# claserken/SISS

Hardware: AMD Instinct MI355X
Metric: unlearning samples/sec (= unlearning-steps/sec x batch x gpus), CelebA-HQ-256 DDPM SISS (higher is better)
Workload: dtype bf16; 1 GPU; delete_celeb.yaml: CelebA-HQ 256x256 DDPM UNet (113.7M params), SISS lambd=0.5, t=999, bf16, bs=16/GPU, GA=1, scaling_norm=500, AdamW lr 5e-6; loss_fn=importance_sampling_with_mixture, global_batch=16, grad_accum=1, parallelism=dp1, hipgraph=True

## Files before the change

### include/siss_hip.h

```cpp
#ifndef SISS_HIP_H
#define SISS_HIP_H
#include <stdint.h>
#ifdef __cplusplus
extern "C" {
#endif

typedef struct siss_tn_job {
    const void* Y; long ldy; const void* X; long ldx; float* dW; long set_stride;
    int N, C, npanels, nsets, rows_per_set, row_begin, row_end, nsplits;
    long x_set_rows;
    const void* zero_page; float* dbias; float* dbias2;
    int shifts[9]; int coffs[9];
    long bias_set_stride;
} siss_tn_job;

typedef struct siss_rk_terms {
    const double* row[8]; double c[8]; int n;
} siss_rk_terms;

long siss_loss_partials_words(int B, long chw);
int siss_mixture_fwd(const void* x0, const void* a0, const void* noise, int in_bf16, const int64_t* t, const
    float* u, const float* alphas_cumprod, const float* gamma_tab, const float* sigma_tab, float lambd, int B,
    long chw, void* x_mix, float* gamma_t, float* sigma_t, float* dist_x, float* dist_a, float* iw_x, float* iw_a,
    double* partials, void* stream);
// ... 71 lines not shown
int siss_groupnorm_set_slab(int on);
long siss_gn_partial_words(int n, int H, int W, int C, int G);
int siss_quad_stats(const void* x, long ld, int M, int N, int rows_per_image, float* qs, void* stream);
int siss_groupnorm_fwd_qs(const void* x, const float* gamma, const float* beta, void* y, float* mean, float*
    rstd, float* partial, const float* qsA, int ca, const float* qsB, int N, int H, int W, int C, int G, float
    eps, int silu, int out_compact, int ldx, void* stream);
int siss_groupnorm_fwd_ld(const void* x, const float* gamma, const float* beta, void* y, float* mean, float*
    rstd, float* partial, int N, int H, int W, int C, int G, float eps, int silu, int out_compact, int ldx, void*
    stream);
int siss_groupnorm_fwd(const void* x, const float* gamma, const float* beta, void* y, float* mean, float*
    rstd, float* partial, int N, int H, int W, int C, int G, float eps, int silu, int out_compact, void* stream);
int siss_groupnorm_bwd_ld(const void* dy, const void* x, const float* gamma, const float* beta, const float*
    mean, const float* rstd, void* dx, const void* accum, const void* accum2, void* dx2, int split_c, int
    accumulate2, float* dgamma, float* dbeta, float* colsum, long colsum_ld, float* partial, int n2, int nx, int
    set_images, long set_stride, int H, int W, int C, int G, int silu, int dy_compact, int ldx, void* stream);
int siss_groupnorm_bwd_ld_s2d(const void* dy, const void* x, const float* gamma, const float* beta, const
    float* mean, const float* rstd, void* dx, const void* accum, const void* accum2, void* dx2, int split_c, int
    accumulate2, float* dgamma, float* dbeta, float* colsum, long colsum_ld, float* partial, int n2, int nx, int
    set_images, long set_stride, int H, int W, int C, int G, int silu, int dy_compact, int ldx, void* stream);
int siss_groupnorm_bwd(const void* dy, const void* x, const float* gamma, const float* beta, const float*
    mean, const float* rstd, void* dx, const void* accum, const void* accum2, void* dx2, int split_c, int
    accumulate2, float* dgamma, float* dbeta, float* colsum, long colsum_ld, float* partial, int n2, int nx, int
    set_images, long set_stride, int H, int W, int C, int G, int silu, int dy_compact, void* stream);

int siss_conv_out_fprop(const void* x, const float* w, const float* bias, float* pred, int B, int H, int W,
    int C, int CO, void* stream);
int siss_conv_out_dgrad(const float* c, const float* w, void* dx, int N2, int H, int W, int C, int CO, void*
    stream);
int siss_conv_out_wgrad(const float* c, const void* x, float* dW, float* dbias, int nsets, int set_images, int
    nx, long set_stride_w, long set_stride_b, int H, int W, int C, int CO, void* stream);
int siss_conv_in_dgrad(const void* dh, long ld, const void* w, int kp, float* dx, int N, int Cin, int H, int
    W, int C0, void* stream);
int siss_conv_in_dgrad_f32(const void* dh, long ld, const void* w, int kp, float* dx, int N, int Cin, int H,
    int W, int C0, void* stream);

int siss_softmax_fwd(const void* s, void* p, long rows, int S, void* stream);
int siss_softmax_bwd(const void* p, const void* dp, void* ds, long rows, long p_rows, int S, float scale,
    void* stream);
int siss_mha_small_takes(int S, int D, int training);
int siss_mha_small_fwd(const void* q, const void* k, const void* v, void* o, float* lse, int N, int S, int C,
    int D, float scale, void* stream);
int siss_mha_small_bwd(const void* q, const void* k, const void* v, const void* o, const float* lse, const
    void* dout, void* dq, void* dk, void* dv, int n2, int nx, int S, int C, int D, float scale, void* stream);
int siss_mha_small_fwd_f32(const void* q, const void* k, const void* v, void* o, float* lse, int N, int S, int
    C, int D, float scale, void* stream);
int siss_mha_small_bwd_f32(const void* q, const void* k, const void* v, const void* o, const float* lse, const
// ... 225 lines not shown
```

### siss_amd/csrc/common.h

```cpp
#pragma once
#include <hip/hip_runtime.h>
#include <stdint.h>

typedef uint16_t bf16_t;

typedef __attribute__((ext_vector_type(8))) short bf16x8_t;
typedef __attribute__((ext_vector_type(4))) float f32x4_t;
typedef __attribute__((ext_vector_type(16))) float f32x16_t;
typedef __attribute__((ext_vector_type(4))) uint32_t u32x4_t;
typedef __attribute__((ext_vector_type(2))) uint32_t u32x2_t;
typedef __attribute__((ext_vector_type(2))) float f32x2_t;
typedef __attribute__((ext_vector_type(2))) __bf16 bf16x2_t;

#define SISS_OK 0
#define SISS_ERR_ARG 1
#define SISS_ERR_LAUNCH 2

#define SISS_CHECK_ARG(cond) \
    do {                     \
        if (!(cond)) return SISS_ERR_ARG; \
    } while (0)

#define SISS_LAUNCH_RET()                                 \
    do {                                                  \
// ... 85 lines not shown
__device__ __forceinline__ unsigned lds_addr(const void* p) {
    return (unsigned)(size_t)(__attribute__((address_space(3))) const char*)p;
}

static inline int cdiv(long a, long b) { return (int)((a + b - 1) / b); }

constexpr int kMaxDevices = 64;
constexpr int kQsTileRows = 254, kQsHalfRows = 128;
static inline int siss_current_device() {
    int dev = 0;
    return hipGetDevice(&dev) == hipSuccess && dev >= 0 && dev < kMaxDevices ? dev : -1;
}
static inline int siss_ensure_smem(const void* kernel, int bytes, unsigned char (&done)[kMaxDevices]) {
    const int dev = siss_current_device();
    if (dev < 0) return SISS_ERR_LAUNCH;
    if (!__atomic_load_n(&done[dev], __ATOMIC_ACQUIRE)) {
        if (hipFuncSetAttribute(kernel, hipFuncAttributeMaxDynamicSharedMemorySize, bytes) != hipSuccess) return SISS_ERR_LAUNCH;
        __atomic_store_n(&done[dev], (unsigned char)1, __ATOMIC_RELEASE);
    }
    return SISS_OK;
}

enum SissKernelId { SISS_K_NT = 0, SISS_K_NT_C3P, SISS_K_FLASH_FWD, SISS_K_FLASH_BWD, SISS_K_NT_SPLITK, SISS_K_TN1, SISS_K_TN3,
                    SISS_K_GN_SLAB, SISS_K_GN_QSTATS, SISS_K_FLASH_QSPLIT, SISS_K_ATTN1H_FWD, SISS_K_ATTN1H_BWD, SISS_K_TN_PAIR, SISS_K_FLASH32, SISS_K_FLASH32_FWD, SISS_K_NT_WIDE, SISS_K_COUNT };
void siss_count_dispatch(int kernel_id);
void* siss_workspace(long* bytes);
```

### siss_amd/csrc/groupnorm.hip

```cpp
#include "common.h"

namespace {

constexpr int kStatsDepth = 2;
constexpr int kThreads = 256;
constexpr int kMaxG = 32;
constexpr int kMaxC = 1024;

struct GNShape {
    int H, W, C, G, cpg, lpp, ppi;
    int chunk_px, nchunks;
    int ld, Gf, nslices;
    int ldx;
};

__device__ __forceinline__ long compact_row(int n, int pi, int H, int W) { return (long)n * H * W + pi; }

__device__ __forceinline__ void unpack8(u32x4_t r, float (&v)[8]) {
#pragma unroll
    for (int j = 0; j < 4; ++j) {
        v[2 * j] = __builtin_bit_cast(float, r[j] << 16);
        v[2 * j + 1] = __builtin_bit_cast(float, r[j] & 0xffff0000u);
    }
}
// ... 338 lines not shown
            }
        }
    }
    for (int k = 0; k < SETS; ++k) {
        reduce_slots(a1[k], active, slot, cc, s, red, ch1);
        reduce_slots(a2[k], active, slot, cc, s, red, ch2);
        const int n2 = k * nx + n;
        if (tid < 2 * s.G) {
            const int g = tid >> 1;
            const float* src = (tid & 1) ? ch2 : ch1;
            float t = 0.f;
            for (int c = g * s.cpg; c < (g + 1) * s.cpg; ++c) t += src[c] * gamma[c];
            partial[(((long)n2 * s.nslices + blockIdx.z) * s.nchunks + chunk) * 2 * s.G + tid] = t;
        }
        const long so = (long)(n2 / set_images) * set_stride + c0;
        for (int i = tid; i < s.C; i += kThreads) {
            atomicAdd(dgamma + so + i, ch2[i]);
            atomicAdd(dbeta + so + i, ch1[i]);
        }
        __syncthreads();
    }
}

template <bool SILU, int SETS, bool S2D>
__global__ __launch_bounds__(kThreads) void gn_bwd_apply_kernel(
    const bf16_t* __restrict__ dy, const bf16_t* __restrict__ x, const float* __restrict__ gamma,
    const float* __restrict__ beta, const float* __restrict__ mean, const float* __restrict__ rstd,
    const float* __restrict__ partial, GNShape s, int nx, int dy_compact, const bf16_t* __restrict__ accum,
    const bf16_t* __restrict__ accum2, bf16_t* __restrict__ dx, bf16_t* __restrict__ dx2, int split_c,
    int accumulate2, float* __restrict__ colsum, long colsum_ld, int pchunks) {
    __shared__ float sh_s1[SETS][kMaxG], sh_s2[SETS][kMaxG];
    __shared__ __attribute__((aligned(16))) float red[2048];
    __shared__ float chs[kMaxC];
    const int n = blockIdx.y, chunk = blockIdx.x, tid = threadIdx.x;
    const int c0 = blockIdx.z * s.C, g0 = blockIdx.z * s.G;
    gamma += c0; beta += c0;
    {
        __shared__ float fr[4][64];
        const double cnt = (double)s.H * s.W * s.cpg;
        for (int k = 0; k < SETS; ++k) {
            const int n2 = k * nx + n;
            fold_slab(partial + ((long)n2 * s.nslices + blockIdx.z) * pchunks * 2 * s.G, pchunks, s.G, fr);
            if (tid < s.G) {
                sh_s1[k][tid] = (float)(((double)fr[0][2 * tid] + fr[1][2 * tid] + fr[2][2 * tid] + fr[3][2 * tid]) / cnt);
                sh_s2[k][tid] = (float)(((double)fr[0][2 * tid + 1] + fr[1][2 * tid + 1] + fr[2][2 * tid + 1] + fr[3][2 * tid + 1]) / cnt);
            }
// ... 49 lines not shown
            const unsigned ooff = __umul24(q.row(), ob);
#pragma unroll
            for (int k = 0; k < SETS; ++k) {
                o.d[k] = ld16(dbase[k], doff);
                if (accum) o.a[k] = ld16(abase[k], roff);
                if (accum2) o.b[k] = ld16(bbase[k], roff);
                if (any_oacc) o.c[k] = oacc ? ld16(obase[k], ooff) : u32x4_t{0u, 0u, 0u, 0u};
            }
        };
        PixelWalk w(s, chunk, slot);
        int yy = S2D ? w.pi / s.W : 0;
        const int dyi = S2D ? s.ppi / s.W : 0;
        In nxt;
        if (w.ok()) issue(w, nxt);
        while (w.ok()) {
            const In cur = nxt;
            const unsigned ooff = out_off(w.row(), yy, w.x);
            if (S2D) yy += dyi + (w.x + w.dx >= s.W ? 1 : 0);
            w.next();
            if (w.ok()) issue(w, nxt);
            float v[8], xh[8], dsl[8];
            unpack8(cur.x, v);
#pragma unroll
            for (int e = 0; e < 8; ++e) {
                xh[e] = v[e] * rs[e] - mr[e];
                dsl[e] = (SILU ? dsilu_f(xh[e] * ga[e] + be[e]) : 1.f) * ga[e];
            }
#pragma unroll
            for (int k = 0; k < SETS; ++k) {
                float d[8], o[8];
                unpack8(cur.d[k], d);
#pragma unroll
                for (int e = 0; e < 8; ++e) {
                    const float t = rs[e] * (d[e] * dsl[e] - m1[k][e] - xh[e] * m2[k][e]);
                    cs[k][e] += t;
                    o[e] = t;
                }
                if (accum) {
                    float r[8];
                    unpack8(cur.a[k], r);
#pragma unroll
                    for (int e = 0; e < 8; ++e) o[e] += r[e];
                }
                if (accum2) {
                    float r[8];
                    unpack8(cur.b[k], r);
#pragma unroll
                    for (int e = 0; e < 8; ++e) o[e] += r[e];
                }
                if (any_oacc) {
                    float r[8];
                    unpack8(cur.c[k], r);
#pragma unroll
                    for (int e = 0; e < 8; ++e) o[e] += r[e];
                }
                st16(obase[k], ooff, pack8(o));
            }
        }
    }
    if (colsum) {
        for (int k = 0; k < SETS; ++k) {
            reduce_slots(cs[k], active, slot, cc, s, red, chs);
            for (int i = tid; i < s.C; i += kThreads) atomicAdd(colsum + (long)(k * nx + n) * colsum_ld + c0 + i, chs[i]);
            __syncthreads();
        }
    }
}

constexpr int kBlocksFwd = 768, kBlocksBwd = 512, kBlocksBwdStats = 767;

bool make_shape(int H, int W, int C, int G, GNShape& s, int N = 16, int blocks = kBlocksFwd) {
    if (H <= 0 || W <= 0 || C <= 0 || G <= 0 || G > kMaxG || C % G || C % 8) return false;
    s.H = H; s.W = W; s.ld = C; s.ldx = C; s.Gf = G; s.cpg = C / G;
    int gs = G;
    if (C > kMaxC) {
        int best = 0, best_util = -1;
        gs = 0;
        for (int d = G; d >= 1; --d) {
            if (G % d) continue;
            const int cs = d * s.cpg;
            if (cs > kMaxC || cs % 8) continue;
            const int lpp = cs / 8, util = (kThreads / lpp) * lpp;
            if (util * 10 >= kThreads * 9) { gs = d; break; }
            if (util > best_util) { best_util = util; best = d; }
        }
        if (gs == 0) gs = best;
        if (gs == 0) return false;
// ... 140 lines not shown
                          float* dbeta, float* colsum, long colsum_ld, float* partial, int n2, int nx, int set_images,
                          long set_stride, int H, int W, int C, int G, int silu, int dy_compact, int ldx, void* stream) {
    return gn_bwd_launch(dy, x, gamma, beta, mean, rstd, dx, accum, accum2, dx2, split_c, accumulate2, dgamma, dbeta, colsum, colsum_ld,
                         partial, n2, nx, set_images, set_stride, H, W, C, G, silu, dy_compact, ldx, 0, stream);
}
int siss_groupnorm_bwd_ld_s2d(const void* dy, const void* x, const float* gamma, const float* beta,
                              const float* mean, const float* rstd, void* dx, const void* accum, const void* accum2,
                              void* dx2, int split_c, int accumulate2, float* dgamma,
                              float* dbeta, float* colsum, long colsum_ld, float* partial, int n2, int nx, int set_images,
                              long set_stride, int H, int W, int C, int G, int silu, int dy_compact, int ldx, void* stream) {
    return gn_bwd_launch(dy, x, gamma, beta, mean, rstd, dx, accum, accum2, dx2, split_c, accumulate2, dgamma, dbeta, colsum, colsum_ld,
                         partial, n2, nx, set_images, set_stride, H, W, C, G, silu, dy_compact, ldx, 1, stream);
}
int siss_groupnorm_bwd(const void* dy, const void* x, const float* gamma, const float* beta,
                       const float* mean, const float* rstd, void* dx, const void* accum, const void* accum2,
                       void* dx2, int split_c, int accumulate2, float* dgamma,
                       float* dbeta, float* colsum, long colsum_ld, float* partial, int n2, int nx, int set_images,
                       long set_stride, int H, int W, int C, int G, int silu, int dy_compact, void* stream) {
    return siss_groupnorm_bwd_ld(dy, x, gamma, beta, mean, rstd, dx, accum, accum2, dx2, split_c, accumulate2, dgamma, dbeta,
                                 colsum, colsum_ld, partial, n2, nx, set_images, set_stride, H, W, C, G, silu, dy_compact, 0,
                                 stream);
}

}
```

### siss_amd/lib.py

```python
import ctypes as C
import os
import re
import threading

import torch

from . import prof

_HERE = os.path.dirname(os.path.abspath(__file__))
LIB_PATH = os.environ.get("SISS_LIB_PATH") or os.path.join(_HERE, "libsiss_hip.so")

P, I, L, D = C.c_void_p, C.c_int, C.c_long, C.c_double
HEADER = os.path.join(os.path.dirname(_HERE), "include", "siss_hip.h")
_SCALARS = {"int": C.c_int, "long": C.c_long, "float": C.c_float, "double": C.c_double}


def parse_prototypes(text):
    text = " ".join(re.sub(r"/\*.*?\*/", " ", text, flags=re.S).split())
    out = {}
    for ret, name, params in re.findall(r"\b(int|long) (siss_\w+) ?\(([^()]*)\) ?;", text):
        out[name] = (_SCALARS[ret], [])
        for decl in ([] if params.strip() in ("", "void") else params.split(",")):
            m = re.fullmatch(r"(?:const )?(\w+)( ?\* ?| )(\w+)", decl.strip())
            if m and "*" in m.group(2):
# ... 32 lines not shown
_MODE = threading.local()


def in_f32_mode():
    return bool(getattr(_MODE, "f32", False))


class f32_mode:

    def __init__(self, on):
        self.on = bool(on)

    def __enter__(self):
        self.prev, _MODE.f32 = getattr(_MODE, "f32", False), self.on
        return self

    def __exit__(self, *exc):
        _MODE.f32 = self.prev
        return False


KERNEL_IDS = {"gemm_nt_kernel": 0, "gemm_nt_c3p_kernel": 1, "flash_attn_fwd": 2, "flash_attn_bwd": 3,
              "gemm_nt_kernel/splitk": 4, "gemm_tn_kernel<1>": 5, "gemm_tn_kernel<3>": 6, "gn_slab": 7, "gn_qstats": 8, "flash_dkdv_qsplit": 9,
              "attn1h_fwd": 10, "attn1h_bwd": 11, "gemm_tn_pair": 12, "flash32_bwd": 13, "flash32_fwd": 14, "gemm_nt_kernel/wide": 15}


def dispatch_counts(reset=False):
    lib = load()
    out = {k: int(lib.siss_dispatch_count(i)) for k, i in KERNEL_IDS.items()}
    if reset:
        lib.siss_dispatch_reset()
    return out



class TNJob(C.Structure):
    _fields_ = [("Y", P), ("ldy", L), ("X", P), ("ldx", L), ("dW", P), ("set_stride", L),
                ("N", I), ("C", I), ("npanels", I), ("nsets", I), ("rows_per_set", I), ("row_begin", I), ("row_end", I),
                ("nsplits", I), ("x_set_rows", L), ("zero_page", P), ("dbias", P), ("dbias2", P),
                ("shifts", I * 9), ("coffs", I * 9), ("bias_set_stride", L)]


class RkTerms(C.Structure):
    _fields_ = [("row", P * 8), ("c", D * 8), ("n", I)]

    @classmethod
    def of(cls, pairs):
# ... 129 lines not shown
```

### siss_amd/prof.py

```python


def _true_rows(M, rows_per_image, Hp, Wp):
    if Hp > 2 and Wp > 2 and M % rows_per_image == 0:
        return (M // rows_per_image) * (Hp - 2) * (Wp - 2)
    return M


def _triples(shifts, coffs, n):
    return n % 3 == 0 and all(shifts[3 * g + 1] == shifts[3 * g] + 1 and shifts[3 * g + 2] == shifts[3 * g] + 2
                              and coffs[3 * g] == coffs[3 * g + 1] == coffs[3 * g + 2] for g in range(n // 3))


def _nt(a, N=None, npanels=1, batch=1, conv=False, planes=False):
    M, N, Kp = a["M"], a["N"] if N is None else N, a["Kp"]
    rpi, Hp, Wp = (a["rows_per_image"], a["Hp"], a["Wp"]) if conv else (1, 0, 0)
    c3p = (conv and not planes and npanels == 9 and batch == 1 and Kp % 64 == 0 and N % 128 == 0 and rpi >= 256
           and -(-M // 128) * -(-N // 128) >= 256 and _triples(a["shifts"], a["coffs"], 9))
    key = ("M", M, "N", N, "K", Kp, "panels", npanels, "batch", batch) + (("4 planes",) if planes else ())
    return ("siss_gemm_nt", 2.0 * _true_rows(M, rpi, Hp, Wp) * N * Kp * npanels * batch, key,
            "gemm_nt_c3p_kernel" if c3p else "gemm_nt_kernel", None)


def _nt_shortcut(a, outer, inner, folded, tag):
    rows = _true_rows(a["M"], a["rows_per_image"], a["Hp"], a["Wp"])
# ... 26 lines not shown

def _tn_pair(a):
    j3, j1 = _job(a["job3"]._obj), _job(a["job1"]._obj)
    key = ("N", j3["N"], "C", j3["C"], "panels", j3["npanels"], "+ N", j1["N"], "C", j1["C"], "panels", j1["npanels"],
           "rows", j3["row_end"] - j3["row_begin"])
    return None, _tn_flops(j3) + _tn_flops(j1), key, "gemm_tn_mixed_kernel", None


def _attn(products, heads, Sq, Sk, D, one_head=False):
    key = ("B", heads, "S", Sq, "D", D) if one_head else ("BH", heads, "Sq", Sq, "Sk", Sk, "D", D)
    return None, 2.0 * products * heads * Sq * Sk * D, key, None, None


def _gn_fwd(a, name="siss_groupnorm_fwd_ld"):
    return name, 0.0, ("n", a["N"], "H", a["H"], "C", a["C"]), name, 2.0 * 2 * a["N"] * a["H"] * a["W"] * a["C"]


def _gn_bwd(a, name="siss_groupnorm_bwd_ld"):
    passes = 2 + (a["accum"] is not None) + (a["accum2"] is not None)
    return (name, 0.0, ("n2", a["n2"], "H", a["H"], "C", a["C"]), name,
            2.0 * (a["H"] * a["W"] * a["C"]) * (a["nx"] + passes * a["n2"]))


def _hbm(nbytes):
    return None, 0.0, (), None, nbytes


def _conv_nt(a):
    return _nt(a, npanels=a["npanels"], conv=True)


_RULES = {
    "siss_gemm_nt": lambda a: _nt(a, npanels=a["npanels"], batch=a["batch"], conv=True),
    "siss_gemm_nt_qstats": _conv_nt,
    "siss_gemm_nt_d2s": _conv_nt,
    "siss_gemm_nt_d2s_bias": _conv_nt,
    "siss_gemm_nt_d2s_phases": lambda a: _nt(a, npanels=a["phase_p0"][4], conv=True, planes=True),
    "siss_gemm_nt_alpha_cols": _nt,
    "siss_gemm_nt_geglu_bwd": _nt,
    "siss_gemm_nt_geglu_fwd": lambda a: _nt(a, N=2 * a["F"]),
    "siss_conv3x3_sc": lambda a: _nt_shortcut(a, "N", "Kp", "K2", "+1x1 K"),
    "siss_conv3x3_dgrad_sc": lambda a: _nt_shortcut(a, "Kp", "N", "Nx", "+1x1 N"),
    "siss_gemm_nt_mulsub": lambda a: (None, 2.0 * a["M"] * a["N"] * a["Kp"] * a["batch"], (), "gemm_nt_kernel", None),
    "siss_gemm_tn": _tn,
    "siss_gemm_tn_bs": _tn,
    "siss_gemm_tn_grouped": lambda a: _tn_table(a, "gemm_tn_grouped_kernel"),
    "siss_gemm_tn_grouped_capped": lambda a: _tn_table(a, "gemm_tn_grouped_capped_kernel"),
    "siss_gemm_tn_pair": _tn_pair,
    "siss_attn1h_fwd": lambda a: _attn(2, a["B"], a["S"], a["S"], a["D"], one_head=True),
    "siss_attn1h_bwd": lambda a: _attn(5, a["nb"], a["S"], a["S"], a["D"], one_head=True),
    "siss_flash_attn_fwd": lambda a: _attn(2, a["BH"], a["Sq_pad"], a["valid_k"], a["D_pad"]),
    "siss_flash_attn_bwd": lambda a: _attn(5, a["nBH"], a["Sq_pad"], a["valid_k"], a["D_pad"]),
    "siss_flash_attn_fwd_merged": lambda a: _attn(2, a["B"] * a["H"], a["Sq"], a["Sk"], a["D"]),
    "siss_flash_attn_bwd_merged": lambda a: _attn(5, a["nB"] * a["H"], a["Sq"], a["Sk"], a["D"]),
    "siss_groupnorm_fwd": lambda a: _gn_fwd(a, None),
    "siss_groupnorm_fwd_ld": _gn_fwd,
    "siss_groupnorm_fwd_qs": _gn_fwd,
    "siss_groupnorm_bwd": lambda a: _gn_bwd(a, None),
    "siss_groupnorm_bwd_ld": _gn_bwd,
    "siss_groupnorm_bwd_ld_s2d": _gn_bwd,
    "siss_recombine_clip_adamw": lambda a: _hbm(32.0 * a["n"]),
    "siss_mixture_fwd": lambda a: _hbm(4.0 * (2 if a["in_bf16"] else 4) * a["B"] * a["chw"]),
    "siss_loss_bwd_seed": lambda a: _hbm((4 + 3 * (2 if a["in_bf16"] else 4) + 8.0) * a["B"] * a["chw"]),
}


def account(name, a):
    booked, work, key, symbol, nbytes = _RULES[name](a) if name in _RULES else (None, 0.0, (), None, None)
    base = booked or name
    base = base[:-3] if base.endswith("_ld") else base
    return base[:-7] if base.endswith("_merged") else base, work, key, symbol or booked or name, nbytes
```

### siss_amd/unet.py

```python
import math
from dataclasses import dataclass
from types import SimpleNamespace

import torch

from . import lib, ops
from .config import UNet2DConfig
from .layout import Act, ActView

ALIGN = 64


@dataclass
class PSpec:
    name: str
    kind: str
    ref_shape: tuple
    native_shape: tuple
    off: int
    numel: int


class ParamStore:

# ... 84 lines not shown
            if n not in sd:
                continue
            t = sd[n]
            if tuple(t.shape) != sp.ref_shape:
                raise ValueError(f"{n}: shape {tuple(t.shape)} != {sp.ref_shape}")
            self.flat[sp.off:sp.off + sp.numel] = self.to_native(sp, t.to(self.flat.device)).reshape(-1)

    def state_dict(self):
        return {n: self.from_native(sp, self.flat[sp.off:sp.off + sp.numel]).cpu() for n, sp in self.specs.items()}

    def grads_ref(self, which):
        return {n: self.from_native(sp, self.grads[which, sp.off:sp.off + sp.numel]).cpu()
                for n, sp in self.specs.items()}

    def flat_to_ref(self, flat):
        return {n: self.from_native(sp, flat[sp.off:sp.off + sp.numel]).cpu() for n, sp in self.specs.items()}


class UNetEngine:
    epi_stats = True
    d2s_epilogue = True
    direct_cat = True
    fold_shortcut = True
    subpixel_up = True
    subpixel_min_px = 1024
    subpixel_queue = 1
    side_max_batch = 1 << 30
    quad_stats = True
    phase_launch = True
    s2d_from_gn = True
    group_rows = 280000
    group_max = 42
    group_attn = True
    fused_attn = True
    wgrad_side = True
    side_blocks = 128
    side_max_px = 256
    side_follow = 1
    prep_side = True
    pair_top = True
    wgrad_overwrite = False
    fill_grads = True
    sparse_fill = True
    sparse_min_floats = 16384
    pair_min_rows = 280000

    def __init__(self, cfg: UNet2DConfig, device="cuda", dtype=torch.bfloat16, f32_fused=False):
        lib.load()
        self.cfg = cfg
        self.device = torch.device(device)
        assert dtype in (torch.bfloat16, torch.float32)
        self.adt, self.f32 = dtype, dtype == torch.float32
        self.f32_fused = bool(f32_fused) and self.f32
        if self.f32:
            self.epi_stats = False
            if not self.f32_fused:
                self.d2s_epilogue = self.fold_shortcut = False
                self.group_rows = 0
        if self.device.type == "cuda":
            lib.ensure_workspace(self.device)
        self.ps = ParamStore()
        self._declare_params()
        self.ps.relayout(self._grads_final_early)
        self.ps.allocate(self.device, f32=self.f32)
        self._build_temb_tables()
        self.wT = {}
        self._wds = {}
        self._acts = {}
        self._bufs = {}
        self._pool = {}
        self.tape = []
        self.gmap = {}
        self._uid = 0
        self.on_early_grads_final = None
        self._wq, self._held, self._held_release = [], {}, []
        self._pair1 = []
        self._wq_post = []
        self._side, self._side_busy, self._side_held, self._side_release, self._side_mark = None, False, {}, [], None
# ... 374 lines not shown
            yptr = y.data
        ldx = getattr(x, "ld", x.c)
        qa = qb = None
        ca = x.c
        if self.epi_stats:
            parts = getattr(x, "cat_parts", None)
            form = (x.c // G) % 4 == 0 and x.c % G == 0
            if parts is not None:
                sa = self._quad_stats_of(parts[0], form and parts[1].c <= 512 and parts[1].c % 8 == 0)
                sb = self._quad_stats_of(parts[1], form and sa is not None)
                if sa is not None and sb is not None:
                    qa, qb, ca = sa, sb, parts[0].c
            else:
                qa = self._quad_stats_of(x, form)
        if qa is not None:
            lib.call("siss_groupnorm_fwd_qs", x.data, ps.p(pre + ".weight"), ps.p(pre + ".bias"), yptr, mean, rstd,
                     self._gn_partial(x.n, x.h, x.w, x.c), qa, ca, qb, x.n, x.h, x.w, x.c, G, float(eps), int(silu),
                     int(compact_out), 0 if ldx == x.c else ldx)
        else:
            lib.call("siss_groupnorm_fwd_ld", x.data, ps.p(pre + ".weight"), ps.p(pre + ".bias"), yptr, mean, rstd,
                     self._gn_partial(x.n, x.h, x.w, x.c), x.n, x.h, x.w, x.c, G, float(eps), int(silu), int(compact_out),
                     0 if ldx == x.c else ldx)

        def bwd(dy, colsum=None, accum: Act = None, colsum_ld=0, accum2: Act = None, split=None):
            nb = self.nb
            held = accum is not None and self._is_held(accum.buf)
            if accum is not None and not held:
                self._wsync(accum)
            s2d = False
            if split is not None:
                da, db, accb = split[:3]
                s2d = len(split) > 3 and bool(split[3])
                dx, dx2p, split_c = da, db.data, (da.c // 4 if s2d else da.c)
                self._wsync(db)
            else:
                dx = accum if (accum is not None and not held) else self._get(nb, x.h, x.w, x.c)
                dx2p, split_c, accb = None, 0, False
            dyp = dy.data if isinstance(dy, Act) else dy
            lib.call("siss_groupnorm_bwd_ld_s2d" if s2d else "siss_groupnorm_bwd_ld", dyp, x.data, ps.p(pre + ".weight"), ps.p(pre + ".bias"), mean, rstd,
                     dx.data, accum.data if accum is not None else None,
                     accum2.data if accum2 is not None else None, dx2p, split_c, int(accb),
                     ps.g(pre + ".weight", self.gbase), ps.g(pre + ".bias", self.gbase), colsum, colsum_ld,
                     self._gn_partial(nb, x.h, x.w, x.c), nb, x.n, self.set_images, ps.total,
                     x.h, x.w, x.c, G, int(silu), int(not isinstance(dy, Act)), 0 if ldx == x.c else ldx)
            if held and split is None:
                self._put(accum)
            return dx
        return y, bwd

    def conv(self, x: Act, pre, ksize=3, rowbias=None, residual: Act = None, out_name=None, ldrb=None, cat_with=None,
             skip_head=None, want_stats=False, shortcut=None, fprop=True):
        ps = self.ps
        w = ps.sh(pre + ".weight")
        if ksize == 1:
            w = w.view(1, *w.shape)
        co = w.shape[1]
        if not fprop:
            y = None
        elif cat_with is not None and self.direct_cat:
            assert (cat_with.n, cat_with.h, cat_with.w) == (x.n, x.h, x.w)
            if isinstance(cat_with, ActView):
# ... 142 lines not shown

    def resnet(self, x: Act, pre, cat_with=None, skip_head=None):
        ps = self.ps
        cin = x.c
        cout = ps.specs[pre + ".conv1.weight"].ref_shape[0]
        B = x.n
        a1, gn1_b = self.gn(x, pre + ".norm1", True)
        col0, _ = self.temb_cols[pre]
        h, c1_b = self.conv(a1, pre + ".conv1", rowbias=self.tp_all[:, col0:], ldrb=self.temb_ntot, want_stats=True)
        a2, gn2_b = self.gn(h, pre + ".norm2", True)
        has_sc = cin != cout
        if has_sc:
            _, sc_b = self.conv(x, pre + ".conv_shortcut", ksize=1, fprop=False)
            out, c2_b = self.conv(a2, pre + ".conv2", cat_with=cat_with, skip_head=skip_head, want_stats=True,
                                  shortcut=(x, pre + ".conv_shortcut"))
        else:
            out, c2_b = self.conv(a2, pre + ".conv2", residual=x, cat_with=cat_with, skip_head=skip_head, want_stats=True)

        def bwd():
            nb = self.nb
            dout = self._take(out)
            gb = self.gbase
            acc_sc = None
            if has_sc:
                sc_b(dout, bias_grad=False, need_dx=False)
                da2, acc_sc = c2_b(dout, bias_grad2=ps.g(pre + ".conv_shortcut.bias", gb),
                                   sc_dgrad=(pre + ".conv_shortcut", x.c, lambda: self._get(nb, x.h, x.w, x.c)))
            else:
                da2 = c2_b(dout)
            dh = gn2_b(da2, colsum=self.dtp_all[:, col0:], accum=None, colsum_ld=self.temb_ntot)
            self._put(da2)
            da1 = c1_b(dh, bias_grad=False)
            self._put(dh)
            prior = self.gmap.pop(id(x), None)
            if has_sc:
                acc = acc_sc if acc_sc is not None else sc_b(dout, bias_grad=False, wgrad=False)
                self._put(dout)
            else:
                acc = dout
            parts = getattr(x, "cat_parts", None)
            if parts is not None:
                a, b = parts
                s2d = bool(getattr(a, "s2d_cot", False)) and self.gmap.get(id(a)) is None
                da = self._get(nb, a.h // 2, a.w // 2, 4 * a.c) if s2d else self._get(nb, a.h, a.w, a.c)
                accb = self.gmap.get(id(b))
                db = accb if accb is not None else self._get(nb, b.h, b.w, b.c)
                gn1_b(da1, accum=acc, accum2=prior, split=(da, db, accb is not None, s2d))
                self.gmap[id(b)] = db
                self._put(acc)
                self._give(a, da)
                x.cat_done = True
            else:
                dx = gn1_b(da1, accum=acc, accum2=prior)
                self.gmap[id(x)] = dx
            self._put(prior)
            self._put(da1)
        self.tape.append(bwd)
        return out

    def attention(self, x: Act, pre):
        ps = self.ps
        C, B, S = x.c, x.n, x.h * x.w
        D = self.cfg.head_dim(C)
        if (self.fused_attn and not self.f32 and D == C and x.w % 4 == 0 and not isinstance(x, ActView)
                and lib.query("siss_attn1h_takes", S, C)):
            return self._attention_fused(x, pre)
        small = D != C
        assert not small or D in (8, 16, 32), f"attention_head_dim {D} is not covered by the HIP kernels"
        if small:
            self._mha_check(S, D, training=False)
            self._mha_sites.append((S, D))
        scale = D ** -0.5
        rows = B * S
        nm = self._name(pre)
        hn, gn_b = self.gn(x, pre + ".group_norm", False, compact_out=True)
        bb = lambda s, shape: self._buf(nm + s, shape, self.adt)
        q, k, v = bb(".q", (rows, C)), bb(".k", (rows, C)), bb(".v", (rows, C))
# ... 514 lines not shown
        plan = None
        if sparse_key is not None and self.sparse_fill and self.wgrad_overwrite and not self.f32 and lib.has("siss_zero_ranges"):
            sparse_key = (sparse_key,) + self._wgrad_sig()
            self._fill_key = sparse_key
            plan = self._fill_plan = self._fill_plans.get(sparse_key)
        g = self.ps.grads

        def fill():
            if plan is None:
                g.zero_()
            elif plan["n"]:
                lib.call("siss_zero_ranges", g, plan["table"], plan["n"], plan["granules"])

        if beside_forward and self.prep_side and self.device.type == "cuda":
            st = self._side_stream()
            st.wait_stream(torch.cuda.current_stream())
            with torch.cuda.stream(st):
                fill()
            self._prep_pending = True
            return
        fill()

    def _wgrad_sig(self):
        return (self.group_rows, self.group_max, self.group_attn, self.pair_top, self.pair_min_rows, self.fold_shortcut, self.subpixel_up,
                self.subpixel_min_px, self.subpixel_queue, self.fused_attn, self.sparse_min_floats, self.wgrad_side, self.side_follow,
                self.on_early_grads_final is not None)

    def _overwritten(self):
        recs = lib.overwrite_log()
        if recs is None:
            return None
        g = self.ps.grads
        base, end = g.data_ptr(), g.data_ptr() + g.numel() * 4
        return tuple(sorted(((a - base) // 4, n) for a, n in recs if base <= a and a + 4 * n <= end))

    def _check_sparse_fill(self):
        key, plan, self._fill_key, self._fill_plan = self._fill_key, self._fill_plan, None, None
        if key is None:
            return
        got = self._overwritten()
        if plan is not None:
            if got != plan["stretches"]:
                self._fill_plans.clear()
                raise RuntimeError("sparse gradient fill: this backward pass did not overwrite the stretches the fill before it skipped "
                                   f"(key {key!r}: {len(plan['stretches'])} recorded, {0 if got is None else len(got)} now) -- the gradients of "
                                   "this step are invalid; schedule switches changed between steps? (UNetEngine.sparse_fill = False)")
            return
# ... 111 lines not shown
```

Before: 309.4 samples/sec.

## Fuse shortcut 1x1 conv dgrad GEMM into groupnorm backward apply kernel

Adds a groupnorm backward kernel that computes the shortcut 1x1 conv input-gradient GEMM (dout x Wsc) in-tile with MFMA and adds it directly in the GN backward apply epilogue, including split/s2d outputs and the accumulate paths. This replaces materialising the shortcut dgrad as a separate full-size activation and reading it back as an accumulator in GN backward, which saves a large HBM round trip at high-resolution ResNet blocks (>=65536 px). The cost is a more complex kernel with an extra finalize launch and GEMM work done at a fixed tile size that may be less efficient than the dedicated GEMM.

```diff
diff --git a/include/siss_hip.h b/include/siss_hip.h
--- a/include/siss_hip.h
+++ b/include/siss_hip.h
@@ -117,6 +117,11 @@
     mean, const float* rstd, void* dx, const void* accum, const void* accum2, void* dx2, int split_c, int
     accumulate2, float* dgamma, float* dbeta, float* colsum, long colsum_ld, float* partial, int n2, int nx, int
     set_images, long set_stride, int H, int W, int C, int G, int silu, int dy_compact, void* stream);
+int siss_groupnorm_bwd_sc(const void* dy, const void* x, const float* gamma, const float* beta, const float*
+    mean, const float* rstd, void* dx, const void* dout, long ldo, const void* wsc, int K, const void* accum2,
+    void* dx2, int split_c, int accumulate2, float* dgamma, float* dbeta, float* colsum, float* partial, float*
+    gconst, int n2, int nx, int set_images, long set_stride, int H, int W, int C, int G, int silu, int s2d, int
+    ldx, void* stream);
 
 int siss_conv_out_fprop(const void* x, const float* w, const float* bias, float* pred, int B, int H, int W,
     int C, int CO, void* stream);
diff --git a/siss_amd/csrc/common.h b/siss_amd/csrc/common.h
--- a/siss_amd/csrc/common.h
+++ b/siss_amd/csrc/common.h
@@ -131,6 +131,6 @@
 }
 
 enum SissKernelId { SISS_K_NT = 0, SISS_K_NT_C3P, SISS_K_FLASH_FWD, SISS_K_FLASH_BWD, SISS_K_NT_SPLITK, SISS_K_TN1, SISS_K_TN3,
-                    SISS_K_GN_SLAB, SISS_K_GN_QSTATS, SISS_K_FLASH_QSPLIT, SISS_K_ATTN1H_FWD, SISS_K_ATTN1H_BWD, SISS_K_TN_PAIR, SISS_K_FLASH32, SISS_K_FLASH32_FWD, SISS_K_NT_WIDE, SISS_K_COUNT };
+                    SISS_K_GN_SLAB, SISS_K_GN_QSTATS, SISS_K_FLASH_QSPLIT, SISS_K_ATTN1H_FWD, SISS_K_ATTN1H_BWD, SISS_K_TN_PAIR, SISS_K_FLASH32, SISS_K_FLASH32_FWD, SISS_K_NT_WIDE, SISS_K_GN_SC, SISS_K_COUNT };
 void siss_count_dispatch(int kernel_id);
 void* siss_workspace(long* bytes);
diff --git a/siss_amd/csrc/groupnorm.hip b/siss_amd/csrc/groupnorm.hip
--- a/siss_amd/csrc/groupnorm.hip
+++ b/siss_amd/csrc/groupnorm.hip
@@ -1,4 +1,4 @@
-#include "common.h"
+#include "nt_common.h"
 
 namespace {
 
@@ -384,6 +384,17 @@
     }
 }
 
+template <bool SILU>
+__device__ __forceinline__ void gn_bwd_xhat(float v, float rs, float mr, float ga, float be, float& xh, float& dsl) {
+#pragma clang fp contract(off)
+    xh = fmaf(v, rs, -mr);
+    dsl = (SILU ? dsilu_f(fmaf(xh, ga, be)) : 1.f) * ga;
+}
+__device__ __forceinline__ float gn_bwd_t(float d, float dsl, float xh, float rs, float m1, float m2) {
+#pragma clang fp contract(off)
+    return rs * fmaf(-xh, m2, fmaf(d, dsl, -m1));
+}
+
 template <bool SILU, int SETS, bool S2D>
 __global__ __launch_bounds__(kThreads) void gn_bwd_apply_kernel(
     const bf16_t* __restrict__ dy, const bf16_t* __restrict__ x, const float* __restrict__ gamma,
@@ -479,17 +490,14 @@
             float v[8], xh[8], dsl[8];
             unpack8(cur.x, v);
 #pragma unroll
-            for (int e = 0; e < 8; ++e) {
-                xh[e] = v[e] * rs[e] - mr[e];
-                dsl[e] = (SILU ? dsilu_f(xh[e] * ga[e] + be[e]) : 1.f) * ga[e];
-            }
+            for (int e = 0; e < 8; ++e) gn_bwd_xhat<SILU>(v[e], rs[e], mr[e], ga[e], be[e], xh[e], dsl[e]);
 #pragma unroll
             for (int k = 0; k < SETS; ++k) {
                 float d[8], o[8];
                 unpack8(cur.d[k], d);
 #pragma unroll
                 for (int e = 0; e < 8; ++e) {
-                    const float t = rs[e] * (d[e] * dsl[e] - m1[k][e] - xh[e] * m2[k][e]);
+                    const float t = gn_bwd_t(d[e], dsl[e], xh[e], rs[e], m1[k][e], m2[k][e]);
                     cs[k][e] += t;
                     o[e] = t;
                 }
@@ -520,6 +528,231 @@
             reduce_slots(cs[k], active, slot, cc, s, red, chs);
             for (int i = tid; i < s.C; i += kThreads) atomicAdd(colsum + (long)(k * nx + n) * colsum_ld + c0 + i, chs[i]);
             __syncthreads();
+        }
+    }
+}
+
+struct GNSCParams {
+    const bf16_t* A; const bf16_t* Wt;
+    const bf16_t* x; const bf16_t* dy; const bf16_t* accum2;
+    const float* gamma; const float* beta; const f32x4_t* gconst;
+    bf16_t* dx; bf16_t* dx2;
+    long lda, ldx;
+    int K, C, G, cpg, Mset, nx, sets, rpi, H, W, split_c, accumulate2;
+    float inv_wp;
+};
+constexpr int kScTileBytes = 128 * kCRow;
+constexpr int kScSmemBytes = kScTileBytes + 3 * kMaxG * 16;
+
+__global__ __launch_bounds__(kThreads) void gn_bwd_sc_finalize_kernel(const float* __restrict__ partial, int pchunks,
+                                                                      const float* __restrict__ mean, const float* __restrict__ rstd,
+                                                                      int G, int nx, double cnt, f32x4_t* __restrict__ gconst) {
+    __shared__ float fr[4][64];
+    const int n2 = blockIdx.x, tid = threadIdx.x;
+    fold_slab(partial + (long)n2 * pchunks * 2 * G, pchunks, G, fr);
+    if (tid < G) {
+        const int n = n2 % nx;
+        const float s1 = (float)(((double)fr[0][2 * tid] + fr[1][2 * tid] + fr[2][2 * tid] + fr[3][2 * tid]) / cnt);
+        const float s2 = (float)(((double)fr[0][2 * tid + 1] + fr[1][2 * tid + 1] + fr[2][2 * tid + 1] + fr[3][2 * tid + 1]) / cnt);
+        const float r = rstd[(long)n * G + tid];
+        gconst[(long)n2 * G + tid] = f32x4_t{r, mean[(long)n * G + tid] * r, s1, s2};
+    }
+}
+
+template <bool SILU, bool S2D, bool EXTRA>
+__global__ __launch_bounds__(kThreads, 3) void gn_bwd_sc_kernel(const GNSCParams p) {
+    constexpr int BM = 128, kPieces = BM / 8 / 4;
+    extern __shared__ __attribute__((aligned(16))) char smem[];
+    const int tid = threadIdx.x, lane = tid & 63;
+    const int w = __builtin_amdgcn_readfirstlane(tid >> 6);
+    const int wm = w >> 1, wn = w & 1;
+    const int tiles_n = (p.C + BN - 1) / BN, tiles_m = (p.Mset + BM - 1) / BM;
+    const int nwg = tiles_n * tiles_m * p.sets;
+    int bid = blockIdx.x;
+    {
+        const int q = nwg >> 3, r = nwg & 7, xcd = bid & 7, k = bid >> 3;
+        bid = (xcd < r ? xcd * (q + 1) : r * (q + 1) + (xcd - r) * q) + k;
+    }
+    const int tn = bid % tiles_n, ts = bid / tiles_n;
+    const int kset = ts % p.sets, tm = ts / p.sets;
+    const int m0 = tm * BM, n0 = tn * BN;
+    const long set_row0 = (long)kset * p.Mset;
+    const bf16_t* A = p.A + set_row0 * p.lda;
+
+    const bf16_t* asrc[kPieces];
+    const bf16_t* wsrc[kPieces];
+#pragma unroll
+    for (int j = 0; j < kPieces; ++j) {
+        const int row = (w * kPieces + j) * 8 + (lane >> 3);
+        const int lc = (lane & 7) ^ ((row >> 1) & 7);
+        int gr = m0 + row; gr = gr < p.Mset ? gr : p.Mset - 1;
+        asrc[j] = A + (long)gr * p.lda + lc * 8;
+        int gn = n0 + row; gn = gn < p.C ? gn : p.C - 1;
+        wsrc[j] = p.Wt + (long)gn * p.K + lc * 8;
+    }
+    const int rpi = p.rpi;
+    const int img0 = m0 / rpi;
+    f32x4_t* cst = reinterpret_cast<f32x4_t*>(smem + kScTileBytes);
+    if (tid < 3 * p.G) {
+        const int slot = tid / p.G, g = tid - slot * p.G;
+        int img = img0 + slot; img = img < p.nx ? img : p.nx - 1;
+        cst[tid] = p.gconst[(long)(kset * p.nx + img) * p.G + g];
+    }
+    const int chunk = tid & 15, trow = tid >> 4;
+    const int nc = n0 + chunk * 8;
+    const bool cols = nc < p.C;
+    float ga[8], be[8];
+#pragma unroll
+    for (int e = 0; e < 8; ++e) { ga[e] = cols ? p.gamma[nc + e] : 0.f; be[e] = cols ? p.beta[nc + e] : 0.f; }
+
+    f32x4_t acc[4][4];
+#pragma unroll
+    for (int i = 0; i < 4; ++i)
+#pragma unroll
+        for (int j = 0; j < 4; ++j) acc[i][j] = f32x4_t{0.f, 0.f, 0.f, 0.f};
+    const int frow = lane & 15, fq = lane >> 4;
+    int a_off[4], w_off[4];
+#pragma unroll
+    for (int i = 0; i < 4; ++i) {
+        const int ra = wm * 64 + i * 16 + frow;
+        a_off[i] = ra * 128 + ((fq ^ ((ra >> 1) & 7)) << 4);
+        const int rw = wn * 64 + i * 16 + frow;
+        w_off[i] = BM * 128 + rw * 128 + ((fq ^ ((rw >> 1) & 7)) << 4);
+    }
+    const unsigned smem_a = lds_addr(smem);
+    const int steps = p.K / BK;
+    for (int s = 0; s < steps; ++s) {
+        asm volatile("s_waitcnt lgkmcnt(0)" ::: "memory");
+        __builtin_amdgcn_s_barrier();
+#pragma unroll
+        for (int j = 0; j < kPieces; ++j) glds16_asm(asrc[j] + s * BK, smem_a + (w * kPieces + j) * 1024);
+#pragma unroll
+        for (int j = 0; j < kPieces; ++j) glds16_asm(wsrc[j] + s * BK, smem_a + BM * 128 + (w * kPieces + j) * 1024);
+        asm volatile("s_waitcnt vmcnt(0)" ::: "memory");
+        __builtin_amdgcn_s_barrier();
+#pragma unroll
+        for (int kk = 0; kk < 2; ++kk) {
+            bf16x8_t af[4], wf[4];
+#pragma unroll
+            for (int i = 0; i < 4; ++i) af[i] = *reinterpret_cast<const bf16x8_t*>(smem + (a_off[i] ^ (kk << 6)));
+#pragma unroll
+            for (int i = 0; i < 4; ++i) wf[i] = *reinterpret_cast<const bf16x8_t*>(smem + (w_off[i] ^ (kk << 6)));
+#pragma unroll
+            for (int i = 0; i < 4; ++i)
+#pragma unroll
+                for (int j = 0; j < 4; ++j)
+                    acc[i][j] = __builtin_amdgcn_mfma_f32_16x16x32_bf16(wf[i], af[j], acc[i][j], 0, 0, 0);
+        }
+    }
+    asm volatile("s_waitcnt lgkmcnt(0)" ::: "memory");
+    __builtin_amdgcn_s_barrier();
+#pragma unroll
+    for (int j = 0; j < 4; ++j) {
+        const int m = wm * 64 + j * 16 + frow;
+#pragma unroll
+        for (int i = 0; i < 4; ++i) {
+            const int nl = wn * 64 + i * 16 + fq * 4;
+            const f32x4_t v = acc[i][j];
+            *reinterpret_cast<u32x2_t*>(smem + m * kCRow + nl * 2) = u32x2_t{pack_bf2(v[0], v[1]), pack_bf2(v[2], v[3])};
+        }
+    }
+    __syncthreads();
+    if (!cols) return;
+
+    const int b1 = (img0 + 1) * rpi - m0, b2 = b1 + rpi;
+    const int g0 = nc / p.cpg, rem0 = nc - g0 * p.cpg;
+    float rs[8], mr[8], m1[8], m2[8];
+    auto load_consts = [&](int slot) {
+        const f32x4_t* c = cst + slot * p.G;
+        int g = g0, rm = rem0;
+#pragma unroll
+        for (int e = 0; e < 8; ++e) {
+            const f32x4_t v = c[g];
+            rs[e] = v[0]; mr[e] = v[1]; m1[e] = v[2]; m2[e] = v[3];
+            if (++rm == p.cpg) { rm = 0; ++g; }
+        }
+    };
+    int cur_slot = (trow >= b1) + (trow >= b2);
+    load_consts(cur_slot);
+    const int Wp = p.W + 2, Hp = p.H + 2;
+    const int C = p.C;
+    const bool second = p.dx2 != nullptr && nc >= p.split_c;
+    const int ostride = p.dx2 ? (second ? C - p.split_c : p.split_c) : C;
+    const bool oacc = EXTRA && second && p.accumulate2;
+    const bool any_oacc = EXTRA && p.dx2 != nullptr && p.accumulate2;
+    const bool s2d_lane = S2D && !second;
+    bf16_t* const obase = second ? p.dx2 + (nc - p.split_c) : p.dx + nc;
+    const int wl2 = (p.W >> 1) + 2;
+    const long img2 = (long)((p.H >> 1) + 2) * wl2;
+    const bf16_t* const xb = p.x + nc;
+    const bf16_t* const db = p.dy + set_row0 * C + nc;
+    const bf16_t* const bb = (EXTRA && p.accum2) ? p.accum2 + set_row0 * C + nc : nullptr;
+    constexpr int kBatch = EXTRA ? 2 : 4;
+    for (int it0 = 0; it0 < BM / 16; it0 += kBatch) {
+        u32x4_t vx[kBatch], vd[kBatch], vb[EXTRA ? kBatch : 1], vc[EXTRA ? kBatch : 1];
+        bf16_t* dst[kBatch];
+        int state[kBatch];
+        int slot_of[kBatch];
+#pragma unroll
+        for (int q = 0; q < kBatch; ++q) {
+            const int row = (it0 + q) * 16 + trow;
+            const int r = m0 + row;
+            const int slot = (row >= b1) + (row >= b2);
+            slot_of[q] = slot;
+            const int img = img0 + slot;
+            const int rem = r - img * rpi;
+            const int y = (int)(((float)rem + 0.5f) * p.inv_wp), xq = rem - y * Wp;
+            const bool halo = (y == 0) | (y == Hp - 1) | (xq == 0) | (xq == Wp - 1);
+            state[q] = r >= p.Mset ? 0 : (halo ? (s2d_lane ? 0 : 1) : 2);
+            vx[q] = vd[q] = u32x4_t{0u, 0u, 0u, 0u};
+            if (EXTRA) vb[q] = vc[q] = u32x4_t{0u, 0u, 0u, 0u};
+            if (s2d_lane) {
+                const int yy = y - 1, xx = xq - 1;
+                dst[q] = p.dx + nc + (((long)(kset * p.nx + img) * img2 + ((yy >> 1) + 1) * wl2 + (xx >> 1) + 1) * 4 + (((yy & 1) << 1) | (xx & 1))) * p.split_c;
+            } else {
+                dst[q] = obase + (set_row0 + r) * ostride;
+            }
+            if (state[q] == 2) {
+                vx[q] = *reinterpret_cast<const u32x4_t*>(xb + (long)r * p.ldx);
+                vd[q] = *reinterpret_cast<const u32x4_t*>(db + (long)r * C);
+                if (EXTRA && bb) vb[q] = *reinterpret_cast<const u32x4_t*>(bb + (long)r * C);
+                if (EXTRA && oacc) vc[q] = *reinterpret_cast<const u32x4_t*>(dst[q]);
+            }
+        }
+#pragma unroll
+        for (int q = 0; q < kBatch; ++q) {
+            if (state[q] == 0) continue;
+            u32x4_t out = u32x4_t{0u, 0u, 0u, 0u};
+            if (state[q] == 2) {
+                if (slot_of[q] != cur_slot) { cur_slot = slot_of[q]; load_consts(cur_slot); }
+                const int row = (it0 + q) * 16 + trow;
+                float v[8], d[8], pr[8], o[8];
+                unpack8(vx[q], v);
+                unpack8(vd[q], d);
+                unpack8(*reinterpret_cast<const u32x4_t*>(smem + row * kCRow + chunk * 16), pr);
+#pragma unroll
+                for (int e = 0; e < 8; ++e) {
+                    float xh, dsl;
+                    gn_bwd_xhat<SILU>(v[e], rs[e], mr[e], ga[e], be[e], xh, dsl);
+                    o[e] = gn_bwd_t(d[e], dsl, xh, rs[e], m1[e], m2[e]);
+                }
+#pragma unroll
+                for (int e = 0; e < 8; ++e) o[e] += pr[e];
+                if (EXTRA && bb) {
+                    float r8[8];
+                    unpack8(vb[q], r8);
+#pragma unroll
+                    for (int e = 0; e < 8; ++e) o[e] += r8[e];
+                }
+                if (EXTRA && any_oacc) {
+                    float r8[8];
+                    unpack8(vc[q], r8);
+#pragma unroll
+                    for (int e = 0; e < 8; ++e) o[e] += r8[e];
+                }
+                out = pack8(o);
+            }
+            *reinterpret_cast<u32x4_t*>(dst[q]) = out;
         }
     }
 }
@@ -706,4 +939,54 @@
                                  stream);
 }
 
-}
+int siss_groupnorm_bwd_sc(const void* dy, const void* x, const float* gamma, const float* beta, const float* mean,
+                          const float* rstd, void* dx, const void* dout, long ldo, const void* wsc, int K, const void* accum2,
+                          void* dx2, int split_c, int accumulate2, float* dgamma, float* dbeta, float* colsum, float* partial,
+                          float* gconst, int n2, int nx, int set_images, long set_stride, int H, int W, int C, int G, int silu,
+                          int s2d, int ldx, void* stream) {
+    GNShape ss;
+    SISS_CHECK_ARG(!colsum);
+    SISS_CHECK_ARG(dy && x && gamma && beta && mean && rstd && dx && dout && wsc && dgamma && dbeta && partial && gconst);
+    SISS_CHECK_ARG(!s2d || (dx2 && H % 2 == 0 && W % 2 == 0));
+    SISS_CHECK_ARG(n2 > 0 && nx > 0 && set_images > 0 && n2 % set_images == 0 && (n2 == nx || n2 == 2 * nx));
+    SISS_CHECK_ARG(K > 0 && K % BK == 0 && ldo >= K && ldo % 8 == 0);
+    SISS_CHECK_ARG(make_shape(H, W, C, G, ss, nx, kBlocksBwdStats) && ss.nslices == 1);
+    SISS_CHECK_ARG(((uintptr_t)dy | (uintptr_t)x | (uintptr_t)dx | (uintptr_t)dout | (uintptr_t)wsc | (uintptr_t)accum2 | (uintptr_t)dx2 |
+                    (uintptr_t)partial | (uintptr_t)gconst) % 16 == 0);
+    SISS_CHECK_ARG(!dx2 || (split_c > 0 && split_c < C && split_c % 8 == 0));
+    SISS_CHECK_ARG(ldx == 0 || (ldx >= C && ldx % 8 == 0));
+    const long rpi = (long)(H + 2) * (W + 2);
+    SISS_CHECK_ARG(rpi >= 64 && nx * rpi < (1L << 31) - 256);
+    if (ldx) ss.ldx = ldx;
+    hipStream_t st = (hipStream_t)stream;
+    static unsigned char attr_set[2][2][2][kMaxDevices];
+    const bool extra = accum2 != nullptr || (dx2 && accumulate2);
+    const bf16_t* dyp = (const bf16_t*)dy; const bf16_t* xp = (const bf16_t*)x;
+    dim3 grid_s(ss.nchunks, nx, 1);
+#define GN_SC_STATS(SILU, SETS) \
+    gn_bwd_stats_kernel<SILU, SETS><<<grid_s, kThreads, 0, st>>>(dyp, xp, gamma, beta, mean, rstd, ss, nx, 0, set_images, set_stride, partial, dgamma, dbeta)
+    if (n2 == nx) { if (silu) { GN_SC_STATS(true, 1); } else { GN_SC_STATS(false, 1); } }
+    else          { if (silu) { GN_SC_STATS(true, 2); } else { GN_SC_STATS(false, 2); } }
+#undef GN_SC_STATS
+    gn_bwd_sc_finalize_kernel<<<n2, kThreads, 0, st>>>(partial, ss.nchunks, mean, rstd, G, nx, (double)H * W * ss.cpg, (f32x4_t*)gconst);
+    GNSCParams p;
+    p.A = (const bf16_t*)dout; p.Wt = (const bf16_t*)wsc; p.x = xp; p.dy = dyp; p.accum2 = (const bf16_t*)accum2;
+    p.gamma = gamma; p.beta = beta; p.gconst = (const f32x4_t*)gconst; p.dx = (bf16_t*)dx; p.dx2 = (bf16_t*)dx2;
+    p.lda = ldo; p.ldx = ss.ldx; p.K = K; p.C = C; p.G = G; p.cpg = ss.cpg; p.Mset = (int)(nx * rpi); p.nx = nx; p.sets = n2 / nx;
+    p.rpi = (int)rpi; p.H = H; p.W = W; p.split_c = split_c; p.accumulate2 = accumulate2; p.inv_wp = 1.0f / (float)(W + 2);
+    const unsigned blocks = (unsigned)(cdiv(p.Mset, 128) * cdiv(C, BN) * p.sets);
+#define GN_SC_(SILU, S2D_, EX)                                                                                                \
+    do {                                                                                                                      \
+        if (siss_ensure_smem((const void*)gn_bwd_sc_kernel<SILU, S2D_, EX>, kScSmemBytes, attr_set[SILU][S2D_][EX]) != SISS_OK) return SISS_ERR_LAUNCH; \
+        gn_bwd_sc_kernel<SILU, S2D_, EX><<<blocks, kThreads, kScSmemBytes, st>>>(p);                                           \
+    } while (0)
+#define GN_SC(SILU, S2D_) do { if (extra) GN_SC_(SILU, S2D_, true); else GN_SC_(SILU, S2D_, false); } while (0)
+    if (silu) { if (s2d) GN_SC(true, true); else GN_SC(true, false); }
+    else      { if (s2d) GN_SC(false, true); else GN_SC(false, false); }
+#undef GN_SC
+#undef GN_SC_
+    siss_count_dispatch(SISS_K_GN_SC);
+    SISS_LAUNCH_RET();
+}
+
+}
diff --git a/siss_amd/lib.py b/siss_amd/lib.py
--- a/siss_amd/lib.py
+++ b/siss_amd/lib.py
@@ -78,7 +78,8 @@
 
 KERNEL_IDS = {"gemm_nt_kernel": 0, "gemm_nt_c3p_kernel": 1, "flash_attn_fwd": 2, "flash_attn_bwd": 3,
               "gemm_nt_kernel/splitk": 4, "gemm_tn_kernel<1>": 5, "gemm_tn_kernel<3>": 6, "gn_slab": 7, "gn_qstats": 8, "flash_dkdv_qsplit": 9,
-              "attn1h_fwd": 10, "attn1h_bwd": 11, "gemm_tn_pair": 12, "flash32_bwd": 13, "flash32_fwd": 14, "gemm_nt_kernel/wide": 15}
+              "attn1h_fwd": 10, "attn1h_bwd": 11, "gemm_tn_pair": 12, "flash32_bwd": 13, "flash32_fwd": 14, "gemm_nt_kernel/wide": 15,
+              "gn_bwd_sc_kernel": 16}
 
 
 def dispatch_counts(reset=False):
diff --git a/siss_amd/prof.py b/siss_amd/prof.py
--- a/siss_amd/prof.py
+++ b/siss_amd/prof.py
@@ -72,6 +72,14 @@
             2.0 * (a["H"] * a["W"] * a["C"]) * (a["nx"] + passes * a["n2"]))
 
 
+def _gn_bwd_sc(a):
+    px = a["H"] * a["W"]
+    passes = 2 + (a["accum2"] is not None) + bool(a["accumulate2"] and a["dx2"] is not None)
+    key = ("n2", a["n2"], "H", a["H"], "C", a["C"], "K", a["K"])
+    return (None, 2.0 * a["n2"] * px * a["C"] * a["K"], key, "gn_bwd_sc_kernel",
+            2.0 * px * (a["C"] * (a["nx"] + passes * a["n2"]) + a["K"] * a["n2"]))
+
+
 def _hbm(nbytes):
     return None, 0.0, (), None, nbytes
 
@@ -115,8 +123,14 @@
 }
 
 
+_LATER_RULES = {
+    "siss_groupnorm_bwd_sc": _gn_bwd_sc,
+}
+
+
 def account(name, a):
-    booked, work, key, symbol, nbytes = _RULES[name](a) if name in _RULES else (None, 0.0, (), None, None)
+    rule = _RULES.get(name) or _LATER_RULES.get(name)
+    booked, work, key, symbol, nbytes = rule(a) if rule else (None, 0.0, (), None, None)
     base = booked or name
     base = base[:-3] if base.endswith("_ld") else base
     return base[:-7] if base.endswith("_merged") else base, work, key, symbol or booked or name, nbytes
diff --git a/siss_amd/unet.py b/siss_amd/unet.py
--- a/siss_amd/unet.py
+++ b/siss_amd/unet.py
@@ -130,6 +130,8 @@
     d2s_epilogue = True
     direct_cat = True
     fold_shortcut = True
+    sc_in_gn = True
+    sc_in_gn_min_px = 65536
     subpixel_up = True
     subpixel_min_px = 1024
     subpixel_queue = 1
@@ -161,7 +163,7 @@
         self.adt, self.f32 = dtype, dtype == torch.float32
         self.f32_fused = bool(f32_fused) and self.f32
         if self.f32:
-            self.epi_stats = False
+            self.epi_stats = self.sc_in_gn = False
             if not self.f32_fused:
                 self.d2s_epilogue = self.fold_shortcut = False
                 self.group_rows = 0
@@ -582,7 +584,8 @@
                      self._gn_partial(x.n, x.h, x.w, x.c), x.n, x.h, x.w, x.c, G, float(eps), int(silu), int(compact_out),
                      0 if ldx == x.c else ldx)
 
-        def bwd(dy, colsum=None, accum: Act = None, colsum_ld=0, accum2: Act = None, split=None):
+        def bwd(dy, colsum=None, accum: Act = None, colsum_ld=0, accum2: Act = None, split=None, sc=None):
+            assert sc is None or (accum is None and colsum is None and isinstance(dy, Act))
             nb = self.nb
             held = accum is not None and self._is_held(accum.buf)
             if accum is not None and not held:
@@ -597,6 +600,14 @@
                 dx = accum if (accum is not None and not held) else self._get(nb, x.h, x.w, x.c)
                 dx2p, split_c, accb = None, 0, False
             dyp = dy.data if isinstance(dy, Act) else dy
+            if sc is not None:
+                dout, wsc = sc
+                lib.call("siss_groupnorm_bwd_sc", dyp, x.data, ps.p(pre + ".weight"), ps.p(pre + ".bias"), mean, rstd, dx.data,
+                         dout.data, getattr(dout, "ld", dout.c), wsc, dout.c, accum2.data if accum2 is not None else None, dx2p,
+                         split_c, int(accb), ps.g(pre + ".weight", self.gbase), ps.g(pre + ".bias", self.gbase), None,
+                         self._gn_partial(nb, x.h, x.w, x.c), self._buf("gn_sc_const", (nb * G * 4,)), nb, x.n, self.set_images,
+                         ps.total, x.h, x.w, x.c, G, int(silu), int(s2d), 0 if ldx == x.c else ldx)
+                return dx
             lib.call("siss_groupnorm_bwd_ld_s2d" if s2d else "siss_groupnorm_bwd_ld", dyp, x.data, ps.p(pre + ".weight"), ps.p(pre + ".bias"), mean, rstd,
                      dx.data, accum.data if accum is not None else None,
                      accum2.data if accum2 is not None else None, dx2p, split_c, int(accb),
@@ -785,7 +796,12 @@
             dout = self._take(out)
             gb = self.gbase
             acc_sc = None
-            if has_sc:
+            sc_gn = (has_sc and self.sc_in_gn and not self.f32 and x.h * x.w >= self.sc_in_gn_min_px and cout % 64 == 0
+                     and cin % 8 == 0 and cin <= 1024 and lib.has("siss_groupnorm_bwd_sc"))
+            if sc_gn:
+                sc_b(dout, bias_grad=False, need_dx=False)
+                da2 = c2_b(dout, bias_grad2=ps.g(pre + ".conv_shortcut.bias", gb))
+            elif has_sc:
                 sc_b(dout, bias_grad=False, need_dx=False)
                 da2, acc_sc = c2_b(dout, bias_grad2=ps.g(pre + ".conv_shortcut.bias", gb),
                                    sc_dgrad=(pre + ".conv_shortcut", x.c, lambda: self._get(nb, x.h, x.w, x.c)))
@@ -796,7 +812,10 @@
             da1 = c1_b(dh, bias_grad=False)
             self._put(dh)
             prior = self.gmap.pop(id(x), None)
-            if has_sc:
+            sc = None
+            if sc_gn:
+                acc, sc = None, (dout, self.wT[pre + ".conv_shortcut.weight"][0])
+            elif has_sc:
                 acc = acc_sc if acc_sc is not None else sc_b(dout, bias_grad=False, wgrad=False)
                 self._put(dout)
             else:
@@ -808,14 +827,16 @@
                 da = self._get(nb, a.h // 2, a.w // 2, 4 * a.c) if s2d else self._get(nb, a.h, a.w, a.c)
                 accb = self.gmap.get(id(b))
                 db = accb if accb is not None else self._get(nb, b.h, b.w, b.c)
-                gn1_b(da1, accum=acc, accum2=prior, split=(da, db, accb is not None, s2d))
+                gn1_b(da1, accum=acc, accum2=prior, split=(da, db, accb is not None, s2d), sc=sc)
                 self.gmap[id(b)] = db
-                self._put(acc)
+                self._put(dout if sc_gn else acc)
                 self._give(a, da)
                 x.cat_done = True
             else:
-                dx = gn1_b(da1, accum=acc, accum2=prior)
+                dx = gn1_b(da1, accum=acc, accum2=prior, sc=sc)
                 self.gmap[id(x)] = dx
+                if sc_gn:
+                    self._put(dout)
             self._put(prior)
             self._put(da1)
         self.tape.append(bwd)
@@ -1376,7 +1397,8 @@
         fill()
 
     def _wgrad_sig(self):
-        return (self.group_rows, self.group_max, self.group_attn, self.pair_top, self.pair_min_rows, self.fold_shortcut, self.subpixel_up,
+        return (self.group_rows, self.group_max, self.group_attn, self.pair_top, self.pair_min_rows, self.fold_shortcut, self.sc_in_gn,
+                self.sc_in_gn_min_px, self.subpixel_up,
                 self.subpixel_min_px, self.subpixel_queue, self.fused_attn, self.sparse_min_floats, self.wgrad_side, self.side_follow,
                 self.on_early_grads_final is not None)
 
```

Measured after the change: 314.6 samples/sec, median of 6. 1.7% higher.
